# patrickfrey/strusPattern

Measured on AMD Instinct MI355X. Metric: GB/s input text scanned + matches/s, 10k-regex lexer + 10k-rule automaton, higher is better.
Workload: dtype u64; 1 GPU; configs[4] per-GPU shard: 10001 regexes + 10000 token rules, 12288 docs x 64KiB UTF-8 per step (the same 805 MB resident in HBM every step; configs[4] asks 32 GB per GPU: 39 such steps)

## Files before the change

struspattern_amd/csrc/l2_fast_kernel.hip:

```cpp
#include <hip/hip_runtime.h>
#include <stdint.h>
#include "l2_fast.h"
#include "l2_device.h"
#include "wave_scan.h"

using namespace spa;

namespace {

typedef uint16_t u16;
typedef uint8_t u8;

typedef const __attribute__((address_space(4))) FastParams& KP;
__device__ __forceinline__ KP kernelParams() { return *(const __attribute__((address_space(4))) FastParams*)__builtin_amdgcn_kernarg_segment_ptr(); }

#define WAVE_FENCE() __builtin_amdgcn_fence( __ATOMIC_ACQ_REL, "wavefront")

enum {NIL16=0xFFFFu};

#ifdef SPA_PROF
#define PROF_DECL u64 prof_t0 = __builtin_amdgcn_s_memtime()
#define PROF_ADD( SLOT) do { const u64 prof_t1 = __builtin_amdgcn_s_memtime(); w.prof[ SLOT] += prof_t1 - prof_t0; prof_t0 = prof_t1; } while (0)
#else
#define PROF_DECL do {} while (0)
#define PROF_ADD( SLOT) do {} while (0)
#endif

__device__ __forceinline__ u64 lanesBelow() { return (1ull << LANE) - 1ull; }
__device__ __forceinline__ u32 evhash( u32 a)
{
	a += ~(a>>5);
	a +=  (a<<3);
	a ^=  (a>>4);
	return a;
}
__device__ __forceinline__ void st4( void* p, u32 a, u32 b, u32 c, u32 d) { u32x4 v; v.x = a; v.y = b; v.z = c; v.w = d; *(u32x4*)p = v; }
__device__ __forceinline__ uint4 ldu4( const void* p)
{
	uint4 v = ld4( p);
	v.x = uni( v.x); v.y = uni( v.y); v.z = uni( v.z); v.w = uni( v.w);
	return v;
}
__device__ __forceinline__ u32 waveScanOr( u32 v)
{
	v |= (u32)__builtin_amdgcn_update_dpp( 0, (int)v, 0x111, 0xF, 0xF, true);
	v |= (u32)__builtin_amdgcn_update_dpp( 0, (int)v, 0x112, 0xF, 0xF, true);
	v |= (u32)__builtin_amdgcn_update_dpp( 0, (int)v, 0x114, 0xF, 0xF, true);
	v |= (u32)__builtin_amdgcn_update_dpp( 0, (int)v, 0x118, 0xF, 0xF, true);
	v |= (u32)__builtin_amdgcn_update_dpp( 0, (int)v, 0x142, 0xA, 0xF, false);
	v |= (u32)__builtin_amdgcn_update_dpp( 0, (int)v, 0x143, 0xC, 0xF, false);
	return v;
}
__device__ __forceinline__ u32 fromLaneBelow( u32 v)
{
	const u32 t = (u32)__builtin_amdgcn_ds_bpermute( (int)((LANE - 1u) << 2), (int)v);
	return LANE ? t : 0u;
}
__device__ __forceinline__ u32 byteField( u32 c0, u32 c1, u32 c2, u32 c3, u32 h)
{
	const u32 wsel = h >> 2;
	const u32 v = wsel == 0 ? c0 : wsel == 1 ? c1 : wsel == 2 ? c2 : c3;
	return (v >> ((h & 3u)*8)) & 0xFFu;
}
__device__ __forceinline__ void byteInc( u32& c0, u32& c1, u32& c2, u32& c3, u32 h)
{
	const u32 inc = 1u << ((h & 3u)*8), ws = h >> 2;
	c0 += ws == 0 ? inc : 0u; c1 += ws == 1 ? inc : 0u; c2 += ws == 2 ? inc : 0u; c3 += ws == 3 ? inc : 0u;
}

#define FALLBACK( WHY) do { w.err = SPD_FAST_FALLBACK; w.why = (WHY); } while (0)
enum {FB_LEXEMS=1, FB_DISPOSE=2, FB_ITEM_AFTER_RESULT=3, FB_ITEMS=4, FB_STAGED=5, FB_RULES=8, FB_BUCKET_SIZE=9, FB_POSLEXEMS=10};

__device__ __forceinline__ bool endLE( u32 hw, u32 pos) { return (hw & H_ENDZERO) || ((hw >> H_END_SHIFT) & H_END_MASK) != ((pos + 1u) & 0xFFu); }
__device__ __forceinline__ bool endEQ( u32 hw, u32 pos) { return (hw & H_ENDZERO) ? (pos == 0) : (((hw >> H_END_SHIFT) & H_END_MASK) == (pos & 0xFFu)); }
__device__ __forceinline__ u32 withEnd( u32 hw, u32 end) { return (hw & ~((H_END_MASK << H_END_SHIFT) | H_ENDZERO)) | ((end & 0xFFu) << H_END_SHIFT); }

template <bool SMALL> struct FreeId { typedef u8 type; };
template <> struct FreeId<false> { typedef u16 type; };
template <int R, int T>
struct LdsDoc
{
	u32 hot[ R];
	u32 kl[ R];
	u64 ent[ T];
	u32 bsize[ 16];
	u32 bmeta[ 16];
	u16 link[ 3*R];
	typename FreeId<(R <= 256)>::type freeS[ R];
	u16 exp[ FAST_EXPCAP];
	u16 expCnt[ 64];
	u16 list[ FAST_LISTCAP];
	u16 rq[ FAST_RQCAP];
};

struct Wave
{
	u32* sp;
	u32 curpos, timestamp, nInstalled, nAlt, nSignals, nTrig, openLo, openHi;
	u32 freeN, usedL, sFreeN, usedS;
	u32 nDispose, nStaged, nStagedItems, err;
	u32 lbase;
	u32 spill;
	u32 why;
	u32 posLexems;
	u32 stopLex, stopOrd, stopTs;
	u32 bsizeV, bmetaV;
	u32 expCntV;
#ifdef SPA_PROF
	u64 prof[ 12];
#endif
};

template <int R, int T>
struct Engine
{
typedef LdsDoc<R,T> Lds;
typedef __attribute__((address_space(3))) Lds& LR;

template <bool SP> static __device__ __forceinline__ u32 ldHot( LR L, const Wave& w, KP P, u32 r) { if (!SP || r < (u32)R) return L.hot[ r]; return w.sp[ P.spill.oHot + (r - R)]; }
template <bool SP> static __device__ __forceinline__ void stHot( LR L, const Wave& w, KP P, u32 r, u32 v) { if (!SP || r < (u32)R) L.hot[ r] = v; else w.sp[ P.spill.oHot + (r - R)] = v; }
template <bool SP> static __device__ __forceinline__ u32 ldLink( LR L, const Wave& w, KP P, u32 r, u32 j) { if (!SP || r < (u32)R) return (u32)L.link[ 3*r + j]; return w.sp[ P.spill.oLink + 3*(r - R) + j]; }
template <bool SP> static __device__ __forceinline__ void stLink( LR L, const Wave& w, KP P, u32 r, u32 j, u32 v) { if (!SP || r < (u32)R) L.link[ 3*r + j] = (u16)v; else w.sp[ P.spill.oLink + 3*(r - R) + j] = v; }
template <bool SP> static __device__ __forceinline__ void ldLinks( LR L, const Wave& w, KP P, u32 r, u32& l0, u32& l1, u32& l2)
{
	if (!SP || r < (u32)R) { l0 = (u32)L.link[ 3*r]; l1 = (u32)L.link[ 3*r+1]; l2 = (u32)L.link[ 3*r+2]; }
	else { const u32* q = &w.sp[ P.spill.oLink + 3*(r - R)]; l0 = q[0]; l1 = q[1]; l2 = q[2]; }
}
template <bool SP> static __device__ __forceinline__ u32 ldKl( LR L, const Wave& w, KP P, u32 r) { if (!SP || r < (u32)R) return L.kl[ r]; return w.sp[ P.spill.oKi + (r - R)]; }
template <bool SP> static __device__ __forceinline__ void stKl( LR L, const Wave& w, KP P, u32 r, u32 ki, u32 lx)
{ const u32 v = ki | (lx << 20); if (!SP || r < (u32)R) L.kl[ r] = v; else w.sp[ P.spill.oKi + (r - R)] = v; }
static __device__ __forceinline__ u32 keyLexemOf( u32 kl, u32 lbase) { return lbase - ((lbase - (kl >> 20)) & 0xFFFu); }
template <bool SP> static __device__ __forceinline__ u32 ldExp( LR L, const Wave& w, KP P, u32 row, u32 i)
{ const u32 C = (u32)FAST_EXPCAP >> P.expShift; if (!SP || i < C) return (u32)L.exp[ row*C + i]; return w.sp[ P.spill.oExp + row*P.spill.maxRules + (i - C)]; }
template <bool SP> static __device__ __forceinline__ void stExp( LR L, const Wave& w, KP P, u32 row, u32 i, u32 r)
{ const u32 C = (u32)FAST_EXPCAP >> P.expShift; if (!SP || i < C) L.exp[ row*C + i] = (u16)r; else w.sp[ P.spill.oExp + row*P.spill.maxRules + (i - C)] = r; }
template <bool SP> static __device__ __forceinline__ u32 ldEv( LR L, const Wave& w, KP P, u32 h, u32 meta, u32 pos)
{ if (!SP || pos < (meta >> 16)) return (u32)L.ent[ (meta & 0xFFFFu) + pos]; return w.sp[ P.spill.oEnt + 2*(h*FAST_SPILL_BUCKET + pos - (meta >> 16))]; }
template <bool SP> static __device__ __forceinline__ uint2 ldEnt( LR L, const Wave& w, KP P, u32 h, u32 meta, u32 pos)
{ if (!SP || pos < (meta >> 16)) { const u64 v = L.ent[ (meta & 0xFFFFu) + pos]; return make_uint2( (u32)v, (u32)(v >> 32)); } return *(const uint2*)&w.sp[ P.spill.oEnt + 2*(h*FAST_SPILL_BUCKET + pos - (meta >> 16))]; }
template <bool SP> static __device__ __forceinline__ u32 ldTs( LR L, const Wave& w, KP P, u32 h, u32 meta, u32 pos) { return ldEnt<SP>( L, w, P, h, meta, pos).y; }
template <bool SP> static __device__ __forceinline__ void stEnt( LR L, const Wave& w, KP P, u32 h, u32 meta, u32 pos, u32 e, u32 t)
{
	if (!SP || pos < (meta >> 16)) L.ent[ (meta & 0xFFFFu) + pos] = (u64)e | ((u64)t << 32);
	else *(uint2*)&w.sp[ P.spill.oEnt + 2*(h*FAST_SPILL_BUCKET + pos - (meta >> 16))] = make_uint2( e, t);
}
template <bool SP> static __device__ __forceinline__ u32 ldList( LR L, const Wave& w, KP P, u32 i) { if (!SP || i < (u32)FAST_LISTCAP) return (u32)L.list[ i]; return w.sp[ P.spill.oList + i]; }
static __device__ __forceinline__ void pushList( LR L, Wave& w, KP P, u32 i, u32 r)
{
	if (i < (u32)FAST_LISTCAP) { if (LANE == 0) L.list[ i] = (u16)r; }
	else { w.spill = 1; if (LANE == 0) w.sp[ P.spill.oList + i] = r; }
}

enum {STAGED_LINE=0x80000000u};
static __device__ __forceinline__ void stageLineResult( Wave& w, KP P, u32 at, u32 ki, u32 startLex, u32 endLex, u32 nStatic, u32 hasNew, u32 newVar, u32 keyLex)
{
	u32* S = &w.sp[ P.spill.oStaged + 8*at];
	st4( S, (u32)STAGED_LINE | ki, 0u, startLex, endLex);
	*(uint2*)(S+4) = make_uint2( nStatic | (hasNew << 2) | (newVar << 8), keyLex);
}
static __device__ __forceinline__ void stageResult( Wave& w, KP P, u32 at, u32 handle, u32 fmt, u32 startLex, u32 endLex, u32 nItems, u32 vars, u32 i0, u32 i1, u32 i2)
{
	u32* S = &w.sp[ P.spill.oStaged + 8*at];
	st4( S, handle, fmt, startLex, endLex);
	st4( S+4, nItems | (vars << 8), i0, i1, i2);
}

template <bool SP>
static __device__ __forceinline__ void fireSignal( LR L, Wave& w, KP P, u32 tsv, u32 sord)
{
	const u32 tid = tsv & 0xFFFFu, r = tid >> 2;
	const u32 sigval = (tsv >> 16) & 0xFu, sigtype = (tsv >> 20) & 0x7u, hasVar = (tsv >> 23) & 1u, variable = tsv >> 24;
	u32 hw = uni( ldHot<SP>( L, w, P, r));
	w.nSignals += 1;
	u32 value = hw & H_VALUE_MASK, count = (hw >> H_COUNT_SHIFT) & H_COUNT_MASK;
	bool match = false, take = false, fin = false;
	switch (sigtype)
	{
		case SIG_ANY:
			take = true;
			if (count > 0) { match = true; --count; fin = (count == 0); hw = withEnd( hw, sord+1); }
			break;
		case SIG_SEQUENCE:
		case SIG_SEQUENCE_IMM:
			if (sigval == value && (sigtype == SIG_SEQUENCE ? endLE( hw, sord) : endEQ( hw, sord)))
			{
				hw = withEnd( hw, sord+1); value = sigval-1;
				if (count > 0) { --count; match = (count == 0); } else match = true;
				fin = (value == 0); take = true;
			}
			break;
		case SIG_WITHIN:
			if ((sigval & value) != 0 && endLE( hw, sord))
			{
				hw = withEnd( hw, sord+1); value &= ~sigval;
				if (count > 0) { --count; match = (count == 0); } else match = true;
				take = true;
			}
			break;
		default:
			hw &= ~(H_VALUE_MASK | (H_COUNT_MASK << H_COUNT_SHIFT));
			if (!(hw & H_LISTED))
			{
				if (w.nDispose < P.spill.maxRules) { pushList( L, w, P, w.nDispose, r); w.nDispose += 1; hw |= H_LISTED; } else FALLBACK( FB_DISPOSE);
			}
			if (LANE == 0) stHot<SP>( L, w, P, r, hw);
			return;
	}
	const bool done = (hw & H_DONE) != 0;
	u32 nItems = (hw >> H_NITEMS_SHIFT) & H_NITEMS_MASK;
	bool newItem = false, newStart = false;
	if (take)
	{
		if (hasVar && P.io.withItems)
		{
			if (done)
			{
				if (nItems) { FALLBACK( FB_ITEM_AFTER_RESULT); return; }
			}
			else if (nItems < 3u) newItem = true;
			else { FALLBACK( FB_ITEMS); return; }
		}
		newStart = !(hw & H_HASSTART);
	}
	if (!done && match && !(hw & H_COLD))
	{
		if (hw & H_VISIBLE)
		{
			if (w.nStaged < P.spill.maxStaged)
			{
				const u32 kl = uni( ldKl<SP>( L, w, P, r)), lx = keyLexemOf( kl, w.lbase);
				if (LANE == 0) stageLineResult( w, P, w.nStaged, kl & 0xFFFFFu, newStart ? w.lbase : lx, w.lbase, nItems, newItem ? 1u : 0u, variable, lx);
				w.nStaged += 1; w.nStagedItems += nItems + (newItem ? 1u : 0u);
			}
			else FALLBACK( FB_STAGED);
		}
		if (newItem) ++nItems;
	}
	else if (!done && (match || newItem || newStart))
	{
		u32* cold = &w.sp[ P.spill.oCold + 8*r];
		u32 handle, fmt, startLex, it0, it1, it2;
		if (hw & H_COLD)
		{
			const uint4 c0 = ldu4( cold), c1 = ldu4( cold + 4);
			handle = c0.x; fmt = c0.y; startLex = c0.z; it0 = c0.w; it1 = c1.x; it2 = c1.y;
		}
		else
		{
			const u32 kl = uni( ldKl<SP>( L, w, P, r)), lx = keyLexemOf( kl, w.lbase);
			const u32* K = (const u32*)&P.keyinst[ kl & 0xFFFFFu];
			handle = ldu( K); fmt = ldu( K+1);
			const u32 vars = ldu( K+14);
			startLex = lx;
			it0 = lx | ((vars & 0xFFu) << 24); it1 = lx | (((vars >> 8) & 0xFFu) << 24); it2 = lx | (((vars >> 16) & 0xFFu) << 24);
		}
		if (newItem)
		{
// ... 147 lines not shown
			const u32 ib = nItemsOut == 3 ? it1 : it0;
			const u32 ic = it0;
			const u32 vars = nItemsOut == 0 ? 0u : nItemsOut == 1 ? (ia >> 24) : nItemsOut == 2 ? ((ia >> 24) | ((ib >> 24) << 8)) : ((ia >> 24) | ((ib >> 24) << 8) | ((ic >> 24) << 16));
			stageResult( w, P, at, handle, fmt, startLex, w.lbase, nItemsOut, vars, ia & 0xFFFFFFu, ib & 0xFFFFFFu, ic & 0xFFFFFFu);
		}
		w.nStaged += nres;
		const u32 itemsIncl = waveScanAdd( (resLine || resRec) ? nItemsOut : 0u);
		w.nStagedItems += (u32)__builtin_amdgcn_readlane( itemsIncl, 63);
	}
	if (recCase && !match)
	{
		st4( cold, handle, fmt, startLex, it0); *(uint2*)(cold + 4) = make_uint2( it1, it2);
		hw |= H_COLD;
	}
	if (nlist)
	{
		if (listNow) L.list[ w.nDispose + (u32)__popcll( listM & lanesBelow())] = (u16)r;
		w.nDispose += nlist;
	}
	if (hit)
	{
		if (listNow) hw |= H_LISTED;
		if (!isDel)
		{
			if (newStart && sord) hw |= H_HASSTART;
			hw = (hw & ~(H_VALUE_MASK | (H_COUNT_MASK << H_COUNT_SHIFT) | (H_NITEMS_MASK << H_NITEMS_SHIFT))) | value | (count << H_COUNT_SHIFT) | ((live ? nItemsOut : nItems) << H_NITEMS_SHIFT);
			if (match && !done) hw |= H_DONE;
		}
		L.hot[ r] = hw & ~(u32)H_MARK;
	}
	WAVE_FENCE();
	return true;
}

template <bool SP>
static __device__ __forceinline__ void deactivateList( LR L, Wave& w, KP P, const u32 nD, const u32 nE, const u32 row)
{
	const u32 n = nD + nE;
	for (u32 base=0; base<n && !w.err; base+=64)
	{
		const u32 nb = (n - base) < 64u ? (n - base) : 64u;
		const bool have = LANE < nb;
		const bool isExp = base + LANE >= nD;
		u32 r = 0, hw = 0;
#if defined(SPA_PROF) && !defined(SPA_PROF_INSTALL)
		u64 pd0 = __builtin_amdgcn_s_memtime();
#define PROF_D( SLOT) do { if (__ballot( hw == 0xFFFFFFFFu)) w.err = SPD_ERR_INTERNAL; const u64 pd1 = __builtin_amdgcn_s_memtime(); w.prof[ SLOT] += pd1 - pd0; pd0 = pd1; } while (0)
#else
#define PROF_D( SLOT) do {} while (0)
#endif
		if (have)
		{
			r = isExp ? ldExp<SP>( L, w, P, row, nE - 1u - (base + LANE - nD)) : ldList<SP>( L, w, P, base + LANE);
			hw = ldHot<SP>( L, w, P, r);
		}
		const bool act = have && (hw & H_ACTIVE) && !(isExp && (hw & H_LISTED));
		const u32 mask = act ? ((hw >> H_TMASK_SHIFT) & H_TMASK_MASK) : 0u;
		if (act) stHot<SP>( L, w, P, r, hw & ~(H_ACTIVE | (H_TMASK_MASK << H_TMASK_SHIFT)));
		if (__ballot( mask != 0))
		{
			u32 lk[ 3] = {0,0,0};
			if (mask) ldLinks<SP>( L, w, P, r, lk[ 0], lk[ 1], lk[ 2]);
#if defined(SPA_PROF) && !defined(SPA_PROF_INSTALL)
			if (__ballot( lk[ 0] == 0xFFFFFFFFu)) w.err = SPD_ERR_INTERNAL;
#endif
			PROF_D( 6);
			const bool slot2 = __ballot( (mask & 4u) != 0) != 0;
			u32 c0 = 0, c1 = 0, c2 = 0, c3 = 0;
#pragma unroll
			for (int j=0; j<2; ++j) if ((mask >> j) & 1u) byteInc( c0, c1, c2, c3, lk[ j] >> 12);
			if (slot2) { if (mask & 4u) byteInc( c0, c1, c2, c3, lk[ 2] >> 12); }
			const u32 i0 = waveScanAdd( c0), i1 = waveScanAdd( c1), i2 = waveScanAdd( c2), i3 = waveScanAdd( c3);
			const u32 e0 = i0 - c0, e1 = i1 - c1, e2 = i2 - c2, e3 = i3 - c3;
			const u32 t0 = (u32)__builtin_amdgcn_readlane( i0, 63), t1 = (u32)__builtin_amdgcn_readlane( i1, 63);
			const u32 t2 = (u32)__builtin_amdgcn_readlane( i2, 63), t3 = (u32)__builtin_amdgcn_readlane( i3, 63);
			const u32 tot = LANE < 16u ? byteField( t0, t1, t2, t3, LANE) : 0u;
			const u32 qoff = waveScanAdd( tot) - tot;
			const u32 total = (u32)__builtin_amdgcn_readlane( qoff + tot, 15);
			if (slot2)
			{
				const u32 h = lk[ 2] >> 12;
				const u32 qo = (u32)__builtin_amdgcn_ds_bpermute( (int)(h << 2), (int)qoff);
				if (mask & 4u) L.rq[ qo + byteField( e0, e1, e2, e3, h)] = (u16)(4u*r + 2u);
			}
#pragma unroll
			for (int j=1; j>=0; --j)
			{
				const u32 h = lk[ j] >> 12;
				const u32 qo = (u32)__builtin_amdgcn_ds_bpermute( (int)(h << 2), (int)qoff);
				if ((mask >> j) & 1u)
				{
					u32 mineBefore = 0;
					if (slot2 && (mask & 4u) && (lk[ 2] >> 12) == h) ++mineBefore;
					if (j == 0 && (mask & 2u) && (lk[ 1] >> 12) == h) ++mineBefore;
					L.rq[ qo + byteField( e0, e1, e2, e3, h) + mineBefore] = (u16)(4u*r + (u32)j);
				}
			}
			WAVE_FENCE();
			PROF_D( 7);
			if (LANE < 16u && tot)
			{
				const u32 h = LANE, meta = w.bmetaV;
				u32 size = w.bsizeV;
				u32 tidNext = (u32)L.rq[ qoff];
				for (u32 q=0; q<tot; ++q)
				{
					const u32 tid = tidNext;
					{ const u32 nx = qoff + q + 1u; tidNext = (u32)L.rq[ nx < (u32)FAST_RQCAP ? nx : (u32)FAST_RQCAP - 1u]; }
					const u32 pos = ldLink<SP>( L, w, P, tid >> 2, tid & 3u) & 0xFFFu;
					const u32 last = size - 1u;
					const uint2 m = ldEnt<SP>( L, w, P, h, meta, last);
					if (!SP || pos != last)
					{
						stEnt<SP>( L, w, P, h, meta, pos, m.x, m.y);
						stLink<SP>( L, w, P, (m.y & 0xFFFFu) >> 2, m.y & 3u, (h << 12) | pos);
					}
					size = last;
					if (SP) WAVE_FENCE();
				}
				L.bsize[ h] = size;
				w.bsizeV = size;
			}
			WAVE_FENCE();
			PROF_D( 11);
			w.nTrig -= total;
#ifdef SPA_PROF
			w.prof[ 8] += (u32)__builtin_amdgcn_readlane( waveScanMax( tot), 63); w.prof[ 9] += 1; w.prof[ 10] += nb;
#endif
		}
		if (nE)
		{
			const bool fr = have && isExp;
			const u64 mL = __ballot( fr && r < (u32)R);
			if (fr && r < (u32)R) L.freeS[ w.freeN + (u32)__popcll( mL & lanesBelow())] = (typename FreeId<(R <= 256)>::type)r;
			w.freeN += (u32)__popcll( mL);
			if (SP)
			{
				const u64 mS = __ballot( fr && r >= (u32)R);
				if (fr && r >= (u32)R) w.sp[ P.spill.oFree + w.sFreeN + (u32)__popcll( mS & lanesBelow())] = r - R;
				w.sFreeN += (u32)__popcll( mS);
			}
		}
		WAVE_FENCE();
	}
}

static __device__ __forceinline__ void setCurrentPos( LR L, Wave& w, KP P, u32 pos)
{
	const u32 W = 1u << P.expShift;
	u32 wcnt = 0;
	while (!w.err)
	{
		u32 n = 0, row = 0;
		while (wcnt < W && w.curpos < pos && !n)
		{
			row = w.curpos & (W-1u);
			n = (u32)__builtin_amdgcn_readlane( w.expCntV, row);
			++wcnt; ++w.curpos;
		}
		u32 nD = w.nDispose;
		if (!n && !nD) break;
		if (nD && n && nD + n > 64u) { n = 0; --wcnt; --w.curpos; }
		w.nDispose = 0;
		if (w.spill) deactivateList<true>( L, w, P, nD, n, row); else deactivateList<false>( L, w, P, nD, n, row);
		if (n)
		{
			if (LANE == 0) L.expCnt[ row] = 0;
			if (LANE == row) w.expCntV = 0;
			WAVE_FENCE();
		}
	}
	if (w.curpos < pos) w.curpos = pos;
	if (w.spill)
	{
		bool over = false;
		if (LANE < 16u) over = w.bsizeV > (w.bmetaV >> 16);
		if (w.expCntV > ((u32)FAST_EXPCAP >> P.expShift)) over = true;
		if (!__ballot( over) && w.sFreeN == w.usedS) { w.spill = 0; w.sFreeN = 0; w.usedS = 0; }
	}
}

template <bool SP>
static __device__ __forceinline__ void installBatchT( LR L, Wave& w, KP P, u32 kb, u32 nb, u32 sord, u64 matMaskIn, u32 rIn,
	const uint4 q0, const uint4 q1, const uint4 q2, const Sim sim)
{
	const u32 value = sim.value, count = sim.count, end = sim.end, startLex = sim.startLex, nItems = sim.nItems, it0 = sim.it0, it1 = sim.it1, it2 = sim.it2;
	const bool hasStart = (sim.flags & S_HASSTART) != 0, done = (sim.flags & S_DONE) != 0, fin = (sim.flags & S_FIN) != 0, del = (sim.flags & S_DEL) != 0, resultNow = (sim.flags & S_RESULT) != 0;
	const bool have = LANE < nb;
	const u32 handle = q0.x, fmt = q0.y, meta = q0.w;
	const u32 tEv[ 3] = {q1.x, q1.z, q2.x};
	const u32 tInfo[ 3] = {q1.y, q1.w, q2.y};
	const u32 range = (meta >> FKI_RANGE_SHIFT) & FKI_RANGE_MASK;
	const u64 matMask = matMaskIn;
	const bool mat = (matMask >> LANE) & 1ull;
	const u32 nmat = (u32)__popcll( matMask);
	const u32 r = rIn;
	if (nmat)
	{
		const u32 row = (sord + range) & ((1u << P.expShift) - 1u);
		u64 same = matMask;
#pragma unroll
		for (int k=0; k<6; ++k)
		{
			const u64 bk = __ballot( mat && ((row >> k) & 1u));
			same &= ((row >> k) & 1u) ? bk : ~bk;
		}
		if (mat)
		{
			const u32 cnt = (u32)L.expCnt[ row];
			stExp<SP>( L, w, P, row, cnt + (u32)__popcll( same & lanesBelow()), r);
			WAVE_FENCE();
			if (!(same >> LANE >> 1)) L.expCnt[ row] = (u16)(cnt + (u32)__popcll( same));
		}
	}
	u32 c0 = 0, c1 = 0, c2 = 0, c3 = 0;
	u32 hB[ 3]; bool inst[ 3];
#pragma unroll
	for (int j=0; j<3; ++j)
	{
		hB[ j] = (tInfo[ j] >> FTI_BUCKET_SHIFT) & 15u;
		inst[ j] = mat && (tInfo[ j] & FTI_INSTALL);
		if (inst[ j]) byteInc( c0, c1, c2, c3, hB[ j]);
	}
	u32 tmask = 0;
	if (__ballot( inst[ 0] || inst[ 1] || inst[ 2]))
	{
		u32 i0 = waveScanAdd( c0), i1 = waveScanAdd( c1), i2 = waveScanAdd( c2), i3 = waveScanAdd( c3);
		const u32 e0 = i0 - c0, e1 = i1 - c1, e2 = i2 - c2, e3 = i3 - c3;
		const u32 t0 = (u32)__builtin_amdgcn_readlane( i0, 63), t1 = (u32)__builtin_amdgcn_readlane( i1, 63);
		const u32 t2 = (u32)__builtin_amdgcn_readlane( i2, 63), t3 = (u32)__builtin_amdgcn_readlane( i3, 63);
		u32 oldSize = 0, add = 0;
		if (LANE < 16u) { oldSize = L.bsize[ LANE]; add = byteField( t0, t1, t2, t3, LANE); }
#pragma unroll
		for (int j=0; j<3; ++j)
		{
			if (inst[ j])
			{
				const u32 h = hB[ j];
				u32 sameB = 0;
#pragma unroll
				for (int jj=0; jj<j; ++jj) if (inst[ jj] && hB[ jj] == h) ++sameB;
				const u32 pos = L.bsize[ h] + byteField( e0, e1, e2, e3, h) + sameB;
				const u32 sv = (tInfo[ j] & FTI_SIGVAL_MASK) | (((tInfo[ j] >> FTI_SIGTYPE_SHIFT) & FTI_SIGTYPE_MASK) << 4) | ((tInfo[ j] & FTI_HASVAR) ? 0x80u : 0u);
				stEnt<SP>( L, w, P, h, L.bmeta[ h], pos, tEv[ j], (4*r + (u32)j) | (sv << 16) | ((tInfo[ j] >> FTI_VAR_SHIFT) << 24));
				stLink<SP>( L, w, P, r, (u32)j, (h << 12) | pos);
				tmask |= 1u << j;
			}
		}
		WAVE_FENCE();
		if (LANE < 16u && add) L.bsize[ LANE] = oldSize + add;
		{
			const u32 s = t0 + t1 + t2 + t3;
			w.nTrig += (s & 0xFFu) + ((s >> 8) & 0xFFu) + ((s >> 16) & 0xFFu) + (s >> 24);
		}
	}
	if (mat)
	{
		u32 hw = value | (count << H_COUNT_SHIFT) | H_ACTIVE | H_COLD | (tmask << H_TMASK_SHIFT) | (nItems << H_NITEMS_SHIFT);
		hw |= end ? ((end & 0xFFu) << H_END_SHIFT) : (u32)H_ENDZERO;
		if (done) hw |= H_DONE;
		if (hasStart) hw |= H_HASSTART;
		if (del || fin) hw |= H_LISTED;
		stHot<SP>( L, w, P, r, hw);
		u32* cold = &w.sp[ P.spill.oCold + 8*r];
		st4( cold, handle, fmt, startLex, it0);
		*(uint2*)(cold + 4) = make_uint2( it1, it2);
	}
	{
		const bool emit = have && resultNow && handle != 0;
		const u64 rm = __ballot( emit);
		if (rm)
		{
			const u32 nr = (u32)__popcll( rm);
			if (w.nStaged + nr > P.spill.maxStaged) { FALLBACK( FB_STAGED); return; }
			if (emit)
			{
				const u32 ia = nItems == 3 ? it2 : nItems == 2 ? it1 : it0;
				const u32 ib = nItems == 3 ? it1 : it0;
				const u32 ic = it0;
				const u32 vars = nItems == 0 ? 0u : nItems == 1 ? (ia >> 24) : nItems == 2 ? ((ia >> 24) | ((ib >> 24) << 8)) : ((ia >> 24) | ((ib >> 24) << 8) | ((ic >> 24) << 16));
				stageResult( w, P, w.nStaged + (u32)__popcll( rm & lanesBelow()), handle, fmt, startLex, w.lbase, nItems, vars, ia & 0xFFFFFFu, ib & 0xFFFFFFu, ic & 0xFFFFFFu);
			}
			w.nStaged += nr;
			u32 incl = waveScanAdd( emit ? nItems : 0u);
			w.nStagedItems += (u32)__builtin_amdgcn_readlane( incl, 63);
		}
	}
	{
		const bool wantDispose = mat && (del || fin);
		const u64 dm = __ballot( wantDispose);
		if (dm)
		{
			const u32 nd = (u32)__popcll( dm);
			if (w.nDispose + nd > P.spill.maxRules) { FALLBACK( FB_DISPOSE); return; }
			if (w.nDispose + nd > (u32)FAST_LISTCAP) w.spill = 1;
			if (wantDispose)
			{
				const u32 at = w.nDispose + (u32)__popcll( dm & lanesBelow());
				if (at < (u32)FAST_LISTCAP) L.list[ at] = (u16)r; else w.sp[ P.spill.oList + at] = r;
			}
			w.nDispose += nd;
		}
	}
	WAVE_FENCE();
}

template <bool SP>
static __device__ __forceinline__ void installStaticT( LR L, Wave& w, KP P, u32 ki0, u32 nb, u32 sord, u32 r,
	const uint4 q0, const uint4 q1, const uint4 q2, const uint4 q3)
{
	const bool have = LANE < nb;
// ... 244 lines not shown
			PROF_I( 11, 0u);
			w.bsizeV = L.bsize[ LANE & 15u];
			continue;
		}
		uint4 q0 = make_uint4( 0,0,0,0), q1 = q0, q2 = q0, q3 = q0;
		if (have)
		{
			const FastKeyInst* K = &P.keyinst[ kb + base + LANE];
			q0 = ld4( K); q1 = ld4( (const u32*)K + 4); q2 = ld4( (const u32*)K + 8); q3 = ld4( (const u32*)K + 12);
		}
		const bool isStatic = (uni( q3.w) & FKF_BATCH_STATIC) != 0 && sord != 0;
		const u32 pastEvent = q0.z, meta = q0.w;
		const u32 tEv[ 3] = {q1.x, q1.z, q2.x};
		const u32 tInfo[ 3] = {q1.y, q1.w, q2.y};
		const u32 range = (meta >> FKI_RANGE_SHIFT) & FKI_RANGE_MASK;
		Sim sim;
		sim.value = meta & FKI_VALUE_MASK; sim.count = (meta >> FKI_COUNT_SHIFT) & FKI_COUNT_MASK; sim.end = 0;
		sim.startLex = 0; sim.nItems = 0; sim.it0 = 0; sim.it1 = 0; sim.it2 = 0; sim.nFires = 0; sim.flags = 0;
		bool dropped = false;
		if (!isStatic && __ballot( have && pastEvent != 0))
		{
			const u32 psi = (have && pastEvent) ? ((meta >> FKI_PASTSTOP_SHIFT) & FKI_PASTSTOP_MASK) : 0u;
			const u32 plex = (u32)__builtin_amdgcn_ds_bpermute( (int)((psi-1u) << 2), (int)w.stopLex);
			const u32 psord = (u32)__builtin_amdgcn_ds_bpermute( (int)((psi-1u) << 2), (int)w.stopOrd);
			const u32 pts = (u32)__builtin_amdgcn_ds_bpermute( (int)((psi-1u) << 2), (int)w.stopTs);
			u32 delTs[ 3];
#pragma unroll
			for (int j=0; j<3; ++j)
			{
				const u32 esi = (tInfo[ j] >> FTI_DELSTOP_SHIFT) & FTI_DELSTOP_MASK;
				delTs[ j] = (u32)__builtin_amdgcn_ds_bpermute( (int)((esi-1u) << 2), (int)w.stopTs);
				if (!esi) delTs[ j] = 0;
			}
			if (psi)
			{
				if (pts && psord + range >= w.curpos)
				{
#pragma unroll
					for (int j=2; j>=0; --j)
					{
						if ((tInfo[ j] & FTI_INSTALL) && tEv[ j] == pastEvent) fireLocal( sim, tInfo[ j], psord, plex, P.io.withItems);
					}
					if (sim.flags & S_DONE) sim.flags |= S_ODD;
					bool cancelled = false;
#pragma unroll
					for (int j=0; j<3; ++j)
					{
						if ((tInfo[ j] & FTI_INSTALL) && ((tInfo[ j] >> FTI_SIGTYPE_SHIFT) & FTI_SIGTYPE_MASK) == SIG_DEL)
						{
							const u32 ts = delTs[ j];
							if (ts && ts > pts) cancelled = true;
						}
					}
					if (cancelled || (sim.flags & (S_DEL | S_FIN))) dropped = true;
				}
			}
			w.nAlt += (u32)__popcll( __ballot( have && pastEvent != 0));
		}
		if (!isStatic)
		{
			if (have && !dropped)
			{
#pragma unroll
				for (int j=0; j<3; ++j) if (tInfo[ j] & FTI_KEY) fireLocal( sim, tInfo[ j], sord, w.lbase, P.io.withItems);
			}
			if (__ballot( (sim.flags & S_ODD) != 0)) { FALLBACK( FB_ITEMS); return; }
		}
		const bool mat = have && !dropped;
		const u64 matMask = __ballot( mat);
		const u32 nmat = (u32)__popcll( matMask);
		w.nInstalled += nb;
		if (isStatic) w.nSignals += (uni( q3.y) >> 8) & 0xFFu;
		else
		{
			u32 incl = waveScanAdd( have ? sim.nFires : 0u);
			w.nSignals += (u32)__builtin_amdgcn_readlane( incl, 63);
		}
		u32 r;
		if (!allocRuleIds( L, w, P, matMask, r)) return;
		if (nmat && !w.spill)
		{
			const u32 row = (sord + range) & ((1u << P.expShift) - 1u);
			const bool over = mat && (u32)L.expCnt[ row] + nmat > ((u32)FAST_EXPCAP >> P.expShift);
			if (__ballot( over)) w.spill = 1;
		}
		{
			bool inst[ 3]; u32 hB[ 3];
#pragma unroll
			for (int j=0; j<3; ++j) { inst[ j] = mat && (tInfo[ j] & FTI_INSTALL); hB[ j] = (tInfo[ j] >> FTI_BUCKET_SHIFT) & 15u; }
			if (!checkBuckets( L, w, P, isStatic ? (uni( q3.y) & 0xFFu) : 3*nmat, inst, hB)) return;
		}
		if (isStatic)
		{
			if (w.spill) installStaticT<true>( L, w, P, kb + base, nb, sord, r, q0, q1, q2, q3);
			else installStaticT<false>( L, w, P, kb + base, nb, sord, r, q0, q1, q2, q3);
		}
		else if (w.spill) installBatchT<true>( L, w, P, kb, nb, sord, matMask, r, q0, q1, q2, sim);
		else installBatchT<false>( L, w, P, kb, nb, sord, matMask, r, q0, q1, q2, sim);
		w.bsizeV = L.bsize[ LANE & 15u];
	}
	w.bsizeV = L.bsize[ LANE & 15u];
	w.expCntV = (u32)L.expCnt[ LANE];
}

template <bool SP>
static __device__ __forceinline__ void scanAndFire( LR L, Wave& w, KP P, u32 id, u32 ordpos)
{
	const u32 h = evhash( id) & 15u;
	const u32 n = (u32)__builtin_amdgcn_readlane( w.bsizeV, h);
	const u32 meta = (u32)__builtin_amdgcn_readlane( w.bmetaV, h);
	for (u32 base=0; base<n && !w.err; base+=64)
	{
		const u32 i = base + LANE;
		uint2 en = make_uint2( 0, 0);
		if (i < n) en = ldEnt<SP>( L, w, P, h, meta, i);
		u64 m = __ballot( i < n && en.x == id);
		if (!SP && (m & (m - 1ull)) != 0)
		{
			if (fireBatch( L, w, P, m, en.y, ordpos)) m = 0;
		}
		while (m && !w.err)
		{
			const u32 p = (u32)__builtin_ctzll( m);
			m &= m-1;
			const u32 tsv = (u32)__builtin_amdgcn_readlane( en.y, p);
			fireSignal<SP>( L, w, P, tsv, ordpos);
		}
	}
}

static __device__ __forceinline__ void runKernel()
{
	KP P = kernelParams();
	__shared__ Lds ldsDoc;
	LR L = *(__attribute__((address_space(3))) Lds*)&ldsDoc;
	Wave w;
	w.sp = P.spillBase + (u64)blockIdx.x * P.spill.totalWords;
	const u32 ndocs = P.io.ndocs;
	const u32 waveSlot = blockIdx.x, nWaveSlots = gridDim.x;

	for (u32 round=0; round<=ndocs; ++round)
	{
		u32 doc = waveSlot;
		if (round)
		{
			u32 nx = 0;
			if (LANE == 0) nx = atomicAdd( P.io.docCursor, 1u);
			doc = nWaveSlots + uni( nx);
		}
		if (doc >= ndocs) break;
		w.bmetaV = P.bucketMeta[ LANE & 15u]; w.bsizeV = 0; w.expCntV = 0;
		if (LANE < 16u) { L.bsize[ LANE] = 0; L.bmeta[ LANE] = w.bmetaV; }
		L.expCnt[ LANE] = 0;
		w.stopLex = 0; w.stopOrd = 0; w.stopTs = 0; w.posLexems = 0;
		w.curpos = 0; w.timestamp = 0; w.nInstalled = 0; w.nAlt = 0; w.nSignals = 0; w.nTrig = 0; w.openLo = 0; w.openHi = 0;
		w.freeN = 0; w.usedL = 0; w.sFreeN = 0; w.usedS = 0;
		w.nDispose = 0; w.nStaged = 0; w.nStagedItems = 0; w.err = 0; w.lbase = 0; w.why = 0; w.spill = 0;
#ifdef SPA_PROF
		for (int pi=0; pi<12; ++pi) w.prof[ pi] = 0;
#endif
		WAVE_FENCE();

		u64 lbeg, lend;
		docLexems( P.io, doc, lbeg, lend);
		if (lend - lbeg >= (1ull << 24)) FALLBACK( FB_LEXEMS);
		u32 curPosition = 0, nEvents = 0;
		for (u64 tile=lbeg; tile<lend && !w.err; tile+=64)
		{
			PROF_DECL;
			uint4 lx = make_uint4( 0,0,0,0); u32 seg = 0;
			const bool mine = tile + LANE < lend;
			if (mine)
			{
				lx = ((const uint4*)P.io.lexems)[ tile + LANE];
				if (P.io.origseg) seg = P.io.origseg[ tile + LANE];
			}
			u32 kBegin = 0, kCount = 0, kStop = 0;
			if (mine && lx.x && lx.x < (1u<<29))
			{
				u32 slot = keyHash( lx.x) & P.keymask;
				for (u32 probes=0; probes<=P.keymask; ++probes)
				{
					const uint4 eq = ld4( &P.keytab[ slot]);
					if (eq.x == lx.x) { kBegin = eq.y; kCount = eq.z; kStop = eq.w; break; }
					if (eq.x == 0) break;
					slot = (slot+1) & P.keymask;
				}
			}
			const u32 cnt = (lend - tile) < 64 ? (u32)(lend - tile) : 64u;
#ifdef SPA_PROF
			if (__ballot( kBegin == 0xFFFFFFFFu)) break;
#endif
			PROF_ADD( 5);
			for (u32 k=0; k<cnt && !w.err; ++k)
			{
				const u32 id = __builtin_amdgcn_readlane( lx.x, k), ordpos = __builtin_amdgcn_readlane( lx.y, k);
				const u32 origpos = __builtin_amdgcn_readlane( lx.z, k), origsize = __builtin_amdgcn_readlane( lx.w, k);
				const u32 origseg = __builtin_amdgcn_readlane( seg, k);
				if (curPosition > ordpos) { w.err = SPD_ERR_ORDER; break; }
				else if (curPosition < ordpos) { curPosition = ordpos; w.posLexems = 0; }
				else if (origsize >= 0x7FFFFFFFu || origseg >= 0x7FFFFFFFu || origpos >= 0x7FFFFFFFu) { w.err = SPD_ERR_RANGE; break; }
				if (w.curpos != ordpos || w.nDispose) { setCurrentPos( L, w, P, ordpos); PROF_ADD( 3); if (w.err) break; }
				if (id >= (1u<<29)) { w.err = SPD_ERR_RANGE; break; }
				w.lbase = (u32)(tile - lbeg) + k;
				if (++w.posLexems > 60u) { FALLBACK( FB_POSLEXEMS); break; }
				{
					const u32 lo = w.openLo + w.nTrig;
					if (lo < w.openLo) w.openHi += 1;
					w.openLo = lo;
				}
				const u32 kb = __builtin_amdgcn_readlane( kBegin, k), kc = __builtin_amdgcn_readlane( kCount, k);
				const u32 stopIdx = __builtin_amdgcn_readlane( kStop, k);
				uint4 pc0 = make_uint4( 0,0,0,0), pc1 = pc0;
				if (LANE < kc) { const u32* S = (const u32*)&P.statics[ kb + LANE]; pc0 = ld4( S); pc1 = ld4( S+4); }
				if (id)
				{
					if (w.spill) scanAndFire<true>( L, w, P, id, ordpos); else scanAndFire<false>( L, w, P, id, ordpos);
				}
				PROF_ADD( 0);
				if (w.err) break;
				if (kc) installBatch( L, w, P, kb, kc, ordpos, pc0, pc1);
				PROF_ADD( 1);
				if (w.err) break;
				WAVE_FENCE();
				if (stopIdx)
				{
					if (LANE == stopIdx-1u) { w.stopLex = w.lbase; w.stopOrd = ordpos; w.stopTs = w.timestamp + 1u; }
					w.timestamp += 1;
					WAVE_FENCE();
				}
				PROF_ADD( 2);
				++nEvents;
			}
		}

		PROF_DECL;
		u32 nres = w.err ? 0 : w.nStaged;
		const u32 nitems = (w.err || !P.io.withItems) ? 0 : w.nStagedItems;
		u64 resBase = 0, itemBase = 0;
		if (nres && !reserveOutput( P.io, SPC_RESULTS, nres, resBase)) { w.err = SPD_ERR_OUTPUT; nres = 0; }
		if (nres && nitems && !reserveOutput( P.io, SPC_ITEMS, nitems, itemBase)) { w.err = SPD_ERR_OUTPUT; nres = 0; }
		if (nres)
		{
			WAVE_FENCE();
			u64 ip = itemBase;
			for (u32 base=0; base<nres; base+=64)
			{
				const u32 ri = base + LANE;
				const bool hv = ri < nres;
				uint4 s0 = make_uint4( 0,0,0,0), s1 = s0;
				if (hv) { const u32* S = &w.sp[ P.spill.oStaged + 8*ri]; s0 = ld4( S); s1 = ld4( S+4); }
				if (hv && (s0.x & (u32)STAGED_LINE))
				{
					const u32* K = (const u32*)&P.keyinst[ s0.x & 0xFFFFFu];
					const u32 handle = K[ 0], fmt = K[ 1], vw = K[ 14];
					const u32 nStatic = s1.x & 3u, hasNew = (s1.x >> 2) & 1u, newVar = (s1.x >> 8) & 0xFFu, lx = s1.y, endLex = s0.w;
					u32 vv[ 3] = {0,0,0}, ll[ 3] = {0,0,0};
					u32 n = 0;
					if (hasNew) { vv[ 0] = newVar; ll[ 0] = endLex; n = 1; }
#pragma unroll
					for (int k=2; k>=0; --k)
					{
						if ((u32)k < nStatic)
						{
							const u32 v = (vw >> (8*k)) & 0xFFu;
							if (n == 0) { vv[ 0] = v; ll[ 0] = lx; } else if (n == 1) { vv[ 1] = v; ll[ 1] = lx; } else if (n == 2) { vv[ 2] = v; ll[ 2] = lx; }
							++n;
						}
					}
					s0.x = handle; s0.y = fmt;
					s1.x = n | (vv[ 0] << 8) | (vv[ 1] << 16) | (vv[ 2] << 24); s1.y = ll[ 0]; s1.z = ll[ 1]; s1.w = ll[ 2];
				}
				const u32 ni = P.io.withItems ? (s1.x & 0xFFu) : 0u;
				u32 incl = waveScanAdd( ni);
				const u64 mine = ip + (incl - ni);
				if (hv)
				{
					const uint4 a = ((const uint4*)P.io.lexems)[ lbeg + s0.z], z = ((const uint4*)P.io.lexems)[ lbeg + s0.w];
					const u32 sa = P.io.origseg ? P.io.origseg[ lbeg + s0.z] : 0u, sz = P.io.origseg ? P.io.origseg[ lbeg + s0.w] : 0u;
					u32* o = P.io.results + (resBase + ri)*9;
					o[0] = s0.x; o[1] = a.y; o[2] = z.y + 1u; o[3] = sa; o[4] = a.z; o[5] = sz; o[6] = z.z + z.w;
					o[7] = P.io.withItems ? (u32)mine : 0u; o[8] = ni;
					if (P.io.withFormats) P.io.resultFormat[ resBase + ri] = s0.y;
					const u32 il[ 3] = {s1.y, s1.z, s1.w};
#pragma unroll
					for (int q=0; q<3; ++q)
					{
						if ((u32)q < ni)
						{
							const uint4 t = ((const uint4*)P.io.lexems)[ lbeg + il[ q]];
							const u32 st = P.io.origseg ? P.io.origseg[ lbeg + il[ q]] : 0u;
							u32* io = P.io.items + (mine + (u32)q)*7;
							io[0] = (s1.x >> (8 + 8*q)) & 0xFFu; io[1] = t.y; io[2] = t.y + 1u; io[3] = st; io[4] = t.z; io[5] = st; io[6] = t.z + t.w;
							if (P.io.withFormats) { P.io.itemFormat[ 2*(mine + (u32)q)] = 0; P.io.itemFormat[ 2*(mine + (u32)q)+1] = 0; }
						}
					}
				}
				ip += (u32)__builtin_amdgcn_readlane( incl, 63);
			}
		}
		PROF_ADD( 4);
#ifdef SPA_PROF
		if (LANE == 0 && P.prof) for (int pi=0; pi<12; ++pi) atomicAdd( (unsigned long long*)&P.prof[ pi], (unsigned long long)w.prof[ pi]);
#endif
		if (w.err != SPD_FAST_FALLBACK) finishDocument( P.io, doc, resBase, nres, w.nInstalled, w.nAlt, w.nSignals, ((u64)w.openHi << 32) | w.openLo, w.err, nEvents);
		else if (LANE == 0)
		{
			const u32 at = atomicAdd( P.fallbackCount, 1u);
			P.fallbackList[ at] = doc;
			P.io.docRange[ 2*(u64)doc] = 0; P.io.docRange[ 2*(u64)doc+1] = 0;
			P.io.docStatus[ doc] = (int32_t)SPD_FAST_FALLBACK;
			atomicAdd( (unsigned long long*)&P.io.counters[ SPC_HANDOVER], 1ull);
			if (P.diag) { atomicAdd( &P.diag[ 0], 1u); atomicAdd( &P.diag[ w.why & 15u], 1u); }
		}
	}
}
};

}

#ifndef SPA_L2_FAST_WAVES_PER_EU
#define SPA_L2_FAST_WAVES_PER_EU 4
#endif
#define SPA_L2_FAST_OCC __attribute__((amdgpu_waves_per_eu( SPA_L2_FAST_WAVES_PER_EU, SPA_L2_FAST_WAVES_PER_EU)))
#define SPA_FAST_VARIANTS( V) \
	V( s, 192, 312) \
	V( m, 320, 512) \
	V( l, 512, 1024) \
	V( t, 8, 128)		 \
	V( n, 256, 448)
#define SPA_FAST_INSTANCE( X, RR, TT) \
	extern "C" __global__ __launch_bounds__(64) SPA_L2_FAST_OCC void spa_l2_fast_kernel_##X( FastParams kernelArgs) { Engine<RR,TT>::runKernel(); }
SPA_FAST_VARIANTS( SPA_FAST_INSTANCE)

namespace spa {
struct FastVariant { void (*kernel)( FastParams); uint32_t R, T; const char* name; };
#define SPA_FAST_ENTRY( X, RR, TT) {spa_l2_fast_kernel_##X, RR, TT, "spa_l2_fast_kernel_" #X},
static const FastVariant fastVariants[ FAST_VARIANTS] = { SPA_FAST_VARIANTS( SPA_FAST_ENTRY) };
static const FastVariant& fastVariantOf( unsigned variant) { return fastVariants[ variant < FAST_VARIANTS ? variant : FAST_VARIANTS-1]; }

unsigned fastVariantNamed( const char* size)
{
	for (unsigned v=0; v<FAST_VARIANTS; ++v) if (size[ 0] == fastVariants[ v].name[ sizeof("spa_l2_fast_kernel_")-1]) return v;
	return FAST_VARIANTS-1;
}
const char* fastKernelName( unsigned variant) { return fastVariantOf( variant).name; }
void fastCapacities( unsigned variant, uint32_t& R, uint32_t& T) { R = fastVariantOf( variant).R; T = fastVariantOf( variant).T; }
int fastBlocksPerCU( unsigned variant)
{
	int n = 0;
	if (hipOccupancyMaxActiveBlocksPerMultiprocessor( &n, (const void*)fastVariantOf( variant).kernel, 64, 0) != hipSuccess || n < 1) n = 1;
	if (n > 32) n = 32;
	return n;
}
hipError_t launchL2Fast( const FastParams& P, unsigned variant, unsigned nblocks, hipStream_t stream)
{
	hipLaunchKernelGGL( fastVariantOf( variant).kernel, dim3( nblocks), dim3( 64), 0, stream, P);
	return hipGetLastError();
}
}
```

Before: 4.260 GB/s.

## Vectorize per-lexeme validation across the wave and skip empty expiry rows via ballot

Per-lexeme order, range and positions-per-lexeme checks move out of the serial per-event loop. They are now computed for all 64 lanes at once using bpermute to the neighbouring lane and ballots, and the serial loop runs only up to the first failing lexeme, after which that error is applied. setCurrentPos now uses a ballot over the expiry counters, rotated to the current position, to jump straight to the next non-empty row instead of stepping one position at a time. This cuts scalar readlanes and branches in the hot serial loop. The cost is extra cross-lane work per tile and subtle edge-carry logic for position runs that span tiles.

Measured after the change: 4.309 GB/s (median of 6 runs). 1.01x the previous value.

```diff
diff --git a/struspattern_amd/csrc/l2_fast_kernel.hip b/struspattern_amd/csrc/l2_fast_kernel.hip
--- a/struspattern_amd/csrc/l2_fast_kernel.hip
+++ b/struspattern_amd/csrc/l2_fast_kernel.hip
@@ -102,7 +102,6 @@
 	u32 lbase;
 	u32 spill;
 	u32 why;
-	u32 posLexems;
 	u32 stopLex, stopOrd, stopTs;
 	u32 bsizeV, bmetaV;
 	u32 expCntV;
@@ -556,11 +555,21 @@
 	while (!w.err)
 	{
 		u32 n = 0, row = 0;
-		while (wcnt < W && w.curpos < pos && !n)
-		{
-			row = w.curpos & (W-1u);
-			n = (u32)__builtin_amdgcn_readlane( w.expCntV, row);
-			++wcnt; ++w.curpos;
+		if (wcnt < W && w.curpos < pos)
+		{
+			const u32 ahead = (pos - w.curpos) < (W - wcnt) ? (pos - w.curpos) : (W - wcnt);
+			const u32 s = w.curpos & (W-1u);
+			u64 em = __ballot( w.expCntV != 0);
+			em = (em >> s) | ((em << 1) << (W - 1u - s));
+			em &= ~0ull >> (64u - ahead);
+			u32 step = ahead;
+			if (em)
+			{
+				step = (u32)__builtin_ctzll( em) + 1u;
+				row = (s + step - 1u) & (W-1u);
+				n = (u32)__builtin_amdgcn_readlane( w.expCntV, row);
+			}
+			wcnt += step; w.curpos += step;
 		}
 		u32 nD = w.nDispose;
 		if (!n && !nD) break;
@@ -1111,7 +1120,7 @@
 		w.bmetaV = P.bucketMeta[ LANE & 15u]; w.bsizeV = 0; w.expCntV = 0;
 		if (LANE < 16u) { L.bsize[ LANE] = 0; L.bmeta[ LANE] = w.bmetaV; }
 		L.expCnt[ LANE] = 0;
-		w.stopLex = 0; w.stopOrd = 0; w.stopTs = 0; w.posLexems = 0;
+		w.stopLex = 0; w.stopOrd = 0; w.stopTs = 0;
 		w.curpos = 0; w.timestamp = 0; w.nInstalled = 0; w.nAlt = 0; w.nSignals = 0; w.nTrig = 0; w.openLo = 0; w.openHi = 0;
 		w.freeN = 0; w.usedL = 0; w.sFreeN = 0; w.usedS = 0;
 		w.nDispose = 0; w.nStaged = 0; w.nStagedItems = 0; w.err = 0; w.lbase = 0; w.why = 0; w.spill = 0;
@@ -1123,7 +1132,7 @@
 		u64 lbeg, lend;
 		docLexems( P.io, doc, lbeg, lend);
 		if (lend - lbeg >= (1ull << 24)) FALLBACK( FB_LEXEMS);
-		u32 curPosition = 0, nEvents = 0;
+		u32 edgePos = 0, edgeRun = 0, nEvents = 0;
 		for (u64 tile=lbeg; tile<lend && !w.err; tile+=64)
 		{
 			PROF_DECL;
@@ -1147,22 +1156,33 @@
 				}
 			}
 			const u32 cnt = (lend - tile) < 64 ? (u32)(lend - tile) : 64u;
+			u32 stop = 0;
+			{
+				const u32 below = (u32)__builtin_amdgcn_ds_bpermute( (int)(((LANE - 1u) & 63u) << 2), (int)lx.y);
+				const u32 prev = LANE ? below : edgePos;
+				const u64 advM = __ballot( mine && prev < lx.y) & (lanesBelow() | (1ull << LANE));
+				const u32 posLexems = advM ? (LANE - (63u - (u32)__builtin_clzll( advM)) + 1u) : ((u32)__builtin_amdgcn_readfirstlane( edgeRun) + LANE + 1u);
+				if (mine)
+				{
+					if (prev > lx.y) stop = SPD_ERR_ORDER;
+					else if (prev == lx.y && (lx.w >= 0x7FFFFFFFu || seg >= 0x7FFFFFFFu || lx.z >= 0x7FFFFFFFu)) stop = SPD_ERR_RANGE;
+					else if (lx.x >= (1u<<29)) stop = SPD_ERR_RANGE;
+					else if (posLexems > 60u) stop = SPD_FAST_FALLBACK;
+				}
+				edgePos = below;
+				edgeRun = (u32)__builtin_amdgcn_ds_bpermute( (int)(((LANE - 1u) & 63u) << 2), (int)posLexems);
+			}
+			u32 nRun = cnt;
+			{ const u64 stopM = __ballot( stop != 0); if (stopM) nRun = (u32)__builtin_ctzll( stopM); }
 #ifdef SPA_PROF
 			if (__ballot( kBegin == 0xFFFFFFFFu)) break;
 #endif
 			PROF_ADD( 5);
-			for (u32 k=0; k<cnt && !w.err; ++k)
+			for (u32 k=0; k<nRun; ++k)
 			{
 				const u32 id = __builtin_amdgcn_readlane( lx.x, k), ordpos = __builtin_amdgcn_readlane( lx.y, k);
-				const u32 origpos = __builtin_amdgcn_readlane( lx.z, k), origsize = __builtin_amdgcn_readlane( lx.w, k);
-				const u32 origseg = __builtin_amdgcn_readlane( seg, k);
-				if (curPosition > ordpos) { w.err = SPD_ERR_ORDER; break; }
-				else if (curPosition < ordpos) { curPosition = ordpos; w.posLexems = 0; }
-				else if (origsize >= 0x7FFFFFFFu || origseg >= 0x7FFFFFFFu || origpos >= 0x7FFFFFFFu) { w.err = SPD_ERR_RANGE; break; }
 				if (w.curpos != ordpos || w.nDispose) { setCurrentPos( L, w, P, ordpos); PROF_ADD( 3); if (w.err) break; }
-				if (id >= (1u<<29)) { w.err = SPD_ERR_RANGE; break; }
 				w.lbase = (u32)(tile - lbeg) + k;
-				if (++w.posLexems > 60u) { FALLBACK( FB_POSLEXEMS); break; }
 				{
 					const u32 lo = w.openLo + w.nTrig;
 					if (lo < w.openLo) w.openHi += 1;
@@ -1191,6 +1211,15 @@
 				PROF_ADD( 2);
 				++nEvents;
 			}
+			if (!w.err)
+			{
+				const u64 stopM = __ballot( stop != 0);
+				if (stopM)
+				{
+					w.err = (u32)__builtin_amdgcn_readlane( stop, (u32)__builtin_ctzll( stopM));
+					if (w.err == SPD_FAST_FALLBACK) w.why = FB_POSLEXEMS;
+				}
+			}
 		}
 
 		PROF_DECL;
```
